# AY-Liu/Image-Editing-Framework

Measured on AMD Instinct MI355X. Metric: denoising steps/sec (SD1.5 512x512 P2P edit step, UNet batch 4), higher is better.
Workload: dtype f16x3; 1 GPU; sd15 UNet (859.5M params) P2P AttentionRefine edit step, 2 prompts x CFG = batch 4, 64x64 latents (512x512 px), 50-step DDIM, guidance 7.5, cross 0.8 / self 0.4, per-step null-text unconditional embeddings (P2P_NTI, edit_real.py); one independent edit per GPU; precision mode f16x3: fp32 storage; every contraction on split operands: hi + lo fp16 halves of each fp32 element, Ah Bh + Al Bh + Ah Bl =

## Files before the change

### image-editing-framework_amd/csrc/conv_halo_x3p.hip

```cpp
#include "x3p_common.h"

template <int N>
struct IntTag { static constexpr int value = N; };

template <bool UPS>
__global__ __launch_bounds__(768) void conv3x3_halo_x3p_kernel(const IefGemmX3pParams p) {
    constexpr int BM = 256, BN = 80, BK = XP_BK, NW = 8, NL = 4;
    constexpr int TM = 2, TN = 5;
    constexpr int WMAX = 64;
    constexpr int NPA = (BM + 2 * WMAX + 2 + 15) / 16;
    constexpr int APL = NPA * 1024;
    constexpr int AD = 2 * APL + 128;
    constexpr int ZA = 2 * APL;
    constexpr int NPB = BN / 16;
    constexpr int BPL = NPB * 1024, BBUF = 2 * BPL, NSB = 5;
    constexpr int BOFF = 2 * AD, DUMP = BOFF + NSB * BBUF;
    constexpr int LDS_BYTES = DUMP + 1024;
    constexpr int NU = 2 * NPA;
    constexpr int ATAPS = 5, APT = 3;
    static_assert(ATAPS * APT * NL >= NU && 3 * NL >= 2 * NPB, "loader schedule");
    static_assert(LDS_BYTES <= 160 * 1024, "LDS");
    __shared__ __attribute__((aligned(1024))) char smem[LDS_BYTES];

    const int tid = threadIdx.x, lane = tid & 63;
// ... 187 lines not shown
            one_step(IntTag<6>{}, IntTag<1>{}, abuf, abuf_n); one_step(IntTag<7>{}, IntTag<0>{}, abuf, abuf_n);
            one_step(IntTag<8>{}, IntTag<1>{}, abuf, abuf_n);
        }
    }
    asm volatile("s_waitcnt lgkmcnt(0)" ::: "memory");

    const float inv = p.inv_scale;
    if (p.splits > 1) {
        float* slab = p.ws + (long long)blockIdx.y * p.M * p.N;
#pragma unroll
        for (int i = 0; i < TM; ++i) {
            const int m = m0 + wave * 32 + i * 16 + fr;
            if (m >= p.M) continue;
#pragma unroll
            for (int j = 0; j < TN; ++j) {
                const int n = n0 + j * 16 + 4 * fq;
                if (n < p.N) *(f32x4*)(slab + (long long)m * p.N + n) = acc[j][i] * inv;
            }
        }
        return;
    }
#pragma unroll
    for (int i = 0; i < TM; ++i) {
        const int m = m0 + wave * 32 + i * 16 + fr;
        if (m >= p.M) continue;
#pragma unroll
        for (int j = 0; j < TN; ++j) {
            const int n = n0 + j * 16 + 4 * fq;
            if (n < p.N) xp_store(p, acc[j][i] * inv, m, n);
        }
    }
}

int ief_conv_halo_x3p_dispatch(const IefGemmX3pParams& p, hipStream_t st) {
    if (!p.conv || p.stride != 1 || p.pad_hi_only || p.CE1 || p.CE2 || p.Wd < 2 || p.H < 2 || p.geglu) return IEF_ESHAPE;
    if (p.ups) {
        if (p.tile != 12 || p.Wd > 128 || (p.H * p.Wd) % 256 || 256 % p.Wd) return IEF_ESHAPE;
    } else if (p.tile != 11 || p.Wd > 64) return IEF_ESHAPE;
    const int ncb = (p.C1 + p.C2) / XP_BK;
    if (p.splits > ncb) return IEF_ESHAPE;
    const int tiles = ((p.M + 255) / 256) * ((p.N + 79) / 80);
    const int splits = p.splits > 1 ? p.splits : 1;
    if (p.ups) hipLaunchKernelGGL(conv3x3_halo_x3p_kernel<true>, dim3(tiles, splits), dim3(768), 0, st, p);
    else hipLaunchKernelGGL(conv3x3_halo_x3p_kernel<false>, dim3(tiles, splits), dim3(768), 0, st, p);
    IEF_LAUNCH_CHECK();
    return IEF_OK;
}
```

### image-editing-framework_amd/csrc/gemm_x3p.hip

```cpp
#include "ief_common.h"
#include "ief_params.h"
#include "x3_common.h"

#include "x3p_common.h"

template <int BM, int BN, int WAVES_M, int WAVES_N, int NS, int NL, bool CONV>
__global__ __launch_bounds__(64 * (WAVES_M * WAVES_N + NL)) void igemm_x3p_kernel(const IefGemmX3pParams p) {
    constexpr int BK = XP_BK;
    constexpr int NWC = WAVES_M * WAVES_N;
    constexpr int NSW = NL > 0 ? NL : NWC;
    constexpr int PA = BM / 16, PB = BN / 16;
    constexpr int P = 2 * (PA + PB);
    constexpr int G = (P + NSW - 1) / NSW;
    constexpr int WM = BM / WAVES_M, WN = BN / WAVES_N, TM = WM / 16, TN = WN / 16;
    constexpr int SLOT = P * 16 * BK;
    constexpr int DUMP = NS * SLOT;
    static_assert(BM % 16 == 0 && BN % 16 == 0 && WM % 16 == 0 && WN % 16 == 0, "tile");
    static_assert(NS >= 2 && NS <= 4, "ring depth");
    static_assert((NS * SLOT + 512) * 2 <= 160 * 1024, "LDS");
    __shared__ __attribute__((aligned(1024))) half_t smem[NS * SLOT + 512];

    const int tid = threadIdx.x, lane = tid & 63;
    const int wave = __builtin_amdgcn_readfirstlane(tid >> 6);
    const int wr = wave / WAVES_N, wc = wave % WAVES_N;
// ... 388 lines not shown
        xp_store(p, a, m, n);
    }
}

__global__ __launch_bounds__(256) void x3_split_act_kernel(const float* __restrict__ x, half_t* __restrict__ planes, long long plane,
                                                           long long rows, int C4, int ldx, int ldp, float scale) {
    const long long total = rows * C4;
    for (long long i = (long long)blockIdx.x * 256 + threadIdx.x; i < total; i += (long long)gridDim.x * 256) {
        const long long r = i / C4;
        const int c = (int)(i - r * C4) * 4;
        half4 h, l;
        split4(*(const f32x4*)(x + r * ldx + c), scale, h, l);
        half_t* o = planes + r * ldp + c;
        *(half4*)o = h;
        *(half4*)(o + plane) = l;
    }
}
extern "C" int ief_x3_split_act(const float* x, ief_half* planes, long long plane, long long rows, int C, int ldx, int ldp, float scale,
                                void* stream) {
    if (!x || !planes) return IEF_EINVAL;
    if (rows <= 0 || C <= 0 || (C & 3) || (ldx & 3) || (ldp & 3) || (plane & 3) || !(scale > 0.f)) return IEF_ESHAPE;
    if (((uintptr_t)x & 15) || ((uintptr_t)planes & 7)) return IEF_EALIGN;
    long long grid = (rows * (C / 4) + 255) / 256;
    if (grid > 16384) grid = 16384;
    hipLaunchKernelGGL(x3_split_act_kernel, dim3((unsigned)grid), dim3(256), 0, (hipStream_t)stream, x, (half_t*)planes, plane, rows,
                       C / 4, ldx, ldp, scale);
    IEF_LAUNCH_CHECK();
    return IEF_OK;
}

extern "C" int ief_gemm_x3p_tile_bm(int tile) {
    switch (tile) {
        case 1: case 2: case 3: case 7: return 128;
        case 4: case 8: case 11: case 12: return 256;
        case 5: return 64;
        case 6: return 128;
        default: return 0;
    }
}
extern "C" int ief_gemm_x3p_tile_wn(int tile) { return tile == 6 ? 64 : tile == 8 ? 160 : 80; }
extern "C" int ief_gemm_x3p_tile_bn(int tile) {
    switch (tile) {
        case 1: case 2: case 4: case 5: case 7: return 160;
        case 3: case 11: case 12: return 80;
        case 6: return 64;
        case 8: return 320;
        default: return 0;
    }
}

template <int BM, int BN, int WAVES_M, int WAVES_N, int NS, int NL>
static int launch_x3p(const IefGemmX3pParams& p, hipStream_t st) {
    const int tiles = ((p.M + BM - 1) / BM) * ((p.N + BN - 1) / BN);
    const int splits = p.splits > 1 ? p.splits : 1;
    constexpr int NT = 64 * (WAVES_M * WAVES_N + NL);
    if (p.conv) hipLaunchKernelGGL((igemm_x3p_kernel<BM, BN, WAVES_M, WAVES_N, NS, NL, true>), dim3(tiles, splits), dim3(NT), 0, st, p);
    else hipLaunchKernelGGL((igemm_x3p_kernel<BM, BN, WAVES_M, WAVES_N, NS, NL, false>), dim3(tiles, splits), dim3(NT), 0, st, p);
    IEF_LAUNCH_CHECK();
    return IEF_OK;
}

int ief_conv_halo_x3p_dispatch(const IefGemmX3pParams& p, hipStream_t st);

extern "C" int ief_gemm_x3p(const IefGemmX3pParams* pp, void* stream) {
    if (!pp || !pp->A || !pp->W || !pp->zeros || (!pp->Out && !pp->OutP)) return IEF_EINVAL;
    IefGemmX3pParams p = *pp;
    if (p.M <= 0 || p.N <= 0 || p.K <= 0 || (p.K % XP_BK) || (p.N & 3)) return IEF_ESHAPE;
    if (p.rowvec && p.rows_per_batch <= 0) return IEF_ESHAPE;
    if (p.splits > 1 && (!p.ws || p.splits > 64 || p.geglu || p.rstat_out || p.cstat_out)) return IEF_EINVAL;
    if (!(p.inv_scale > 0.f)) return IEF_EINVAL;
    if ((p.ldw & 7) || (p.planeW & 7) || ((uintptr_t)p.W & 15)) return IEF_EALIGN;
    if (p.Out && ((p.ldo & 3) || ((uintptr_t)p.Out & 15))) return IEF_EALIGN;
    if (p.OutP && ((p.ldp & 3) || (p.planeO & 3) || ((uintptr_t)p.OutP & 7))) return IEF_EALIGN;
    if ((p.bias && ((uintptr_t)p.bias & 15)) || (p.rowvec && ((uintptr_t)p.rowvec & 15)) ||
        (p.residual && (((uintptr_t)p.residual & 15) || (p.ldr & 3)))) return IEF_EALIGN;
    if (p.geglu && ((p.N & 15) || p.residual || p.rowvec)) return IEF_EINVAL;
    if (p.rstat_out && (p.splits > 1 || p.geglu || p.tile == 11 || p.tile == 12 || (p.N % ief_gemm_x3p_tile_wn(p.tile)))) return IEF_EINVAL;
    if (p.rstat_in && (!p.colsum || p.rstat_slots <= 0 || p.rstat_cnt <= 0 || p.rstat_slots * p.rstat_cnt != p.K || p.splits > 1 ||
                       p.conv || !(p.ln_eps > 0.f) || ((uintptr_t)p.colsum & 15))) return IEF_EINVAL;
    if (p.conv) {
        if (p.C1 <= 0 || p.C2 < 0 || (p.C1 % XP_BK) || (p.C2 % XP_BK) || (p.CE1 % XP_BK) || (p.CE2 % XP_BK)) return IEF_ESHAPE;
        if ((p.C2 > 0 && !p.A2) || (p.CE1 > 0 && !p.E1) || (p.CE2 > 0 && !p.E2) || (p.CE2 > 0 && p.CE1 == 0)) return IEF_EINVAL;
        if (p.stride != 1 && p.stride != 2) return IEF_ESHAPE;
        if (p.ups != 0 && p.ups != 1) return IEF_ESHAPE;
        if (p.ups && ((p.H | p.Wd) & 1)) return IEF_ESHAPE;
        if ((p.CE1 + p.CE2) > 0 && (p.stride != 1 || p.ups)) return IEF_ESHAPE;
        if (p.K != 9 * (p.C1 + p.C2) + p.CE1 + p.CE2 || p.batch_images <= 0 || p.M != p.batch_images * p.Ho * p.Wo) return IEF_ESHAPE;
        const long long in_pix = (long long)p.batch_images * (p.H >> p.ups) * (p.Wd >> p.ups);
        const int cmax = p.C1 > p.C2 ? p.C1 : p.C2, emax = p.CE1 > p.CE2 ? p.CE1 : p.CE2;
        if (in_pix * cmax * 2 >= (1ll << 32) || (long long)p.M * emax * 2 >= (1ll << 32)) return IEF_ESHAPE;
        if (((uintptr_t)p.A & 15) || (p.planeA & 7) || (p.A2 && (((uintptr_t)p.A2 & 15) || (p.planeA2 & 7))) ||
            (p.E1 && (((uintptr_t)p.E1 & 15) || (p.planeE1 & 7))) || (p.E2 && (((uintptr_t)p.E2 & 15) || (p.planeE2 & 7)))) return IEF_EALIGN;
    } else {
        if ((p.lda & 7) || (p.planeA & 7) || ((uintptr_t)p.A & 15)) return IEF_EALIGN;
    }
    hipStream_t st = (hipStream_t)stream;
    int rc;
    switch (p.tile) {
        case 2: rc = launch_x3p<128, 160, 4, 2, 4, 4>(p, st); break;
        case 3: rc = launch_x3p<128, 80, 4, 1, 3, 0>(p, st); break;
        case 4: rc = launch_x3p<256, 160, 4, 2, 3, 0>(p, st); break;
        case 5: rc = launch_x3p<64, 160, 2, 2, 4, 0>(p, st); break;
        case 6: rc = launch_x3p<128, 64, 4, 1, 3, 0>(p, st); break;
        case 7: rc = launch_x3p<128, 160, 2, 2, 2, 0>(p, st); break;
        case 8: rc = launch_x3p<256, 320, 4, 2, 2, 0>(p, st); break;
        case 11: case 12: rc = ief_conv_halo_x3p_dispatch(p, st); break;
        case 1: default: rc = launch_x3p<128, 160, 4, 2, 4, 0>(p, st); break;
    }
    if (rc) return rc;
    if (p.splits > 1) {
        const long long total = (long long)p.M * (p.N / 4);
        int grid = (int)((total + 255) / 256);
        if (grid > 8192) grid = 8192;
        hipLaunchKernelGGL(x3p_reduce_kernel, dim3(grid), dim3(256), 0, st, p);
        IEF_LAUNCH_CHECK();
    }
    return IEF_OK;
}
```

### image-editing-framework_amd/csrc/split_x3.hip

```cpp
#include "ief_common.h"
#include "ief_params.h"

#include "x3_common.h"

__global__ __launch_bounds__(256) void x3_split_weights_kernel(const float* __restrict__ w, half_t* __restrict__ planes, long long n4,
                                                               float s) {
    for (long long i = (long long)blockIdx.x * 256 + threadIdx.x; i < n4; i += (long long)gridDim.x * 256) {
        half4 h, l;
        split4(((const f32x4*)w)[i], s, h, l);
        ((half4*)planes)[i] = h;
        ((half4*)planes)[n4 + i] = l;
    }
}
extern "C" int ief_x3_split_weights(const float* w, void* planes, long long n, float scale, void* stream) {
    if (!w || !planes) return IEF_EINVAL;
    if (n <= 0 || (n & 3) || !(scale > 0.f)) return IEF_ESHAPE;
    if (((uintptr_t)w & 15) || ((uintptr_t)planes & 7)) return IEF_EALIGN;
    long long grid = (n / 4 + 255) / 256;
    if (grid > 16384) grid = 16384;
    hipLaunchKernelGGL(x3_split_weights_kernel, dim3((unsigned)grid), dim3(256), 0, (hipStream_t)stream, w, (half_t*)planes, n / 4, scale);
    IEF_LAUNCH_CHECK();
    return IEF_OK;
}

template <int WM, int WN, int TM, int TN, int KIND, bool TRANSB, bool BPRE>
__global__ __launch_bounds__(64 * WM * WN, (2 * 2 * 16 * (WM * TM + WN * TN) * YLD * 2 > 80 * 1024) ? (WM * WN) / 4 : (WM * WN) / 2)
void igemm_x3_kernel(const IefGemmF32Params p) {
    constexpr bool CONV = KIND >= X3_CONV;
    constexpr bool HASFAST = KIND == X3_LIN || KIND == X3_CONV;
    constexpr int NTH = 64 * WM * WN;
    constexpr int BM = 16 * WM * TM, BN = 16 * WN * TN;
    constexpr int ROWS = BM + BN;
    constexpr int NA = (BM * 8 + NTH - 1) / NTH;
    constexpr int NBC = BPRE ? 2 * BN * 4 : BN * 8;
    constexpr int NB = (NBC + NTH - 1) / NTH;
    constexpr bool A_EXACT = (BM * 8) % NTH == 0, B_EXACT = NBC % NTH == 0;
    static_assert(!(BPRE && TRANSB), "pre-split planes are [N][K]");
    constexpr unsigned OOB = 0xFFFFFFF0u;
    constexpr unsigned OOBF = 0x80000000u;
    __shared__ __attribute__((aligned(16))) half_t smem_y[2 * 2 * ROWS * YLD];
    const int tid = threadIdx.x, lane = tid & 63, wid = tid >> 6;
    const int wm = wid / WN, wn = wid - wm * WN;
    const int lr = lane & 15, lg = lane >> 4;
    const int ntn = (p.N + BN - 1) / BN;
    const int ntiles = ((p.M + BM - 1) / BM) * ntn;
    const int bid = xcd_remap(blockIdx.x, ntiles);
    const int ntm = (p.M + BM - 1) / BM;
    const int grp = bid / (X3_GROUP_M * ntn), within = bid - grp * (X3_GROUP_M * ntn);
    const int gsz = min(X3_GROUP_M, ntm - grp * X3_GROUP_M);
    const int tn = within / gsz, tm = grp * X3_GROUP_M + (within - tn * gsz);
    const int m0 = tm * BM, n0 = tn * BN;
    const float* A = p.A;
    const float* W = p.W;
// ... 1088 lines not shown
```

### image-editing-framework_amd/hip.py

```python
import ctypes
import os
from ctypes import byref

import torch

from . import cabi

ABI_VERSION = cabi.defines["IEF_ABI_VERSION"]
REPEAT_MAX_JOBS = cabi.defines["IEF_REPEAT_MAX_JOBS"]
_LIB_PATH = os.environ.get("IEF_HIP_LIB") or os.path.join(os.path.dirname(os.path.abspath(__file__)), "libief_hip.so")
_lib = None


class HipExtensionMissing(RuntimeError):
    pass


IefGemmParams = cabi.structs["IefGemmParams"]
IefAttnParams = cabi.structs["IefAttnParams"]
IefCrossParams = cabi.structs["IefCrossParams"]
IefGemmF32Params = cabi.structs["IefGemmF32Params"]
IefAttnF32Params = cabi.structs["IefAttnF32Params"]
IefRepeatJob = cabi.structs["IefRepeatJob"]
IefGemmX3pParams = cabi.structs["IefGemmX3pParams"]
# ... 372 lines not shown
    def __init__(self, mode: str):
        if mode not in ("f32", "x3"):
            raise ValueError('f32_contraction: mode must be "f32" or "x3"')
        self.mode = mode

    def __enter__(self):
        global _F32_CONTRACT
        self.saved, _F32_CONTRACT = _F32_CONTRACT, self.mode
        return self

    def __exit__(self, *exc):
        global _F32_CONTRACT
        _F32_CONTRACT = self.saved
        return False


_x3_planes = {}
X3_FUSE_GEGLU = os.environ.get("IEF_X3_FUSE_GEGLU", "1") == "1"
X3_PRESPLIT = os.environ.get("IEF_X3_PRESPLIT", "1") == "1"


def x3_weight_planes(w, scale=None):
    scale = X3_SCALE_W if scale is None else scale
    key = (w.data_ptr(), tuple(w.shape), float(scale))
    hit = _x3_planes.get(key)
    if hit is not None and hit[0]() is w and hit[1] == w._version:
        return hit[2]
    if _capturing() or w.numel() % 4 or not w.is_contiguous():
        return None
    lib = load()
    n = w.shape[0]
    planes = torch.empty(2, n, w.numel() // n, dtype=torch.float16, device=w.device)
    _check(lib.ief_x3_split_weights(w.data_ptr(), planes.data_ptr(), w.numel(), float(scale), _stream()), "ief_x3_split_weights")
    import weakref
    _x3_planes[key] = (weakref.ref(w), w._version, planes)
    weakref.finalize(w, _x3_planes.pop, key, None)
    return planes


def _set_x3(p, sa, sb, w=None) -> str:
    if _F32_CONTRACT == "x3":
        p.x3, p.sa, p.sb = 1, sa, sb
        if w is not None and X3_PRESPLIT and (w.numel() // w.shape[0]) % 8 == 0:
            planes = x3_weight_planes(w, sb)
            if planes is not None:
                p._planes = planes
                p.Wp = planes.data_ptr()
        return "igemm_x3_kernel"
    return "igemm_f32_kernel"


def _is32(t) -> bool:
    return isinstance(t, torch.Tensor) and t.dtype == torch.float32


def _act32(t, name):
    if not (isinstance(t, torch.Tensor) and t.is_cuda and t.dtype == torch.float32):
        raise TypeError(f"{name}: expected an fp32 device tensor (reference-precision mode), got "
                        f"{type(t).__name__ if not isinstance(t, torch.Tensor) else (t.dtype, t.device)}")
    if t.stride(-1) != 1:
        raise ValueError(f"{name}: last dimension must be contiguous")
    return t


def _rows_ld32(t, name):
    _act32(t, name)
# ... 1555 lines not shown
```

### image-editing-framework_amd/planes.py

```python
import os
from ctypes import byref

import torch

from . import hip
from .hip import IefGemmX3pParams, _check, _dev32, _ptr, _stream, _Timed, _zeros

ACT_SCALE = 1.0
W_SCALE = hip.X3_SCALE_W


class Planes:
    __slots__ = ("t",)

    def __init__(self, t):
        if not (isinstance(t, torch.Tensor) and t.dtype == torch.float16 and t.dim() >= 2 and t.shape[0] == 2 and t.stride(-1) == 1):
            raise TypeError("Planes: expected an fp16 tensor [2, ...] with a contiguous last dimension")
        if not t.is_cuda:
            raise TypeError("Planes: device tensor expected (no CPU path)")
        self.t = t

    @staticmethod
    def empty(*shape, device):
        return Planes(torch.empty(2, *shape, dtype=torch.float16, device=device))
# ... 59 lines not shown
    return out


def weight_planes(w):
    t = hip.x3_weight_planes(w, W_SCALE)
    if t is None:
        raise RuntimeError("weight planes missing while capturing: run one eager forward first")
    return t


_PLAN_FILE = os.environ.get("IEF_PLAN_FILE_X3") or os.path.join(os.path.dirname(os.path.abspath(__file__)), "tuned_plans_x3.json")
_plans = None
TILE_FORCE = int(os.environ.get("IEF_X3P_TILE", "0"))


def _plan_table():
    global _plans
    if _plans is None:
        _plans = {}
        if os.path.exists(_PLAN_FILE) and os.environ.get("IEF_NO_PLAN_TABLE", "0") != "1":
            import json
            with open(_PLAN_FILE) as f:
                _plans = {k: tuple(v) for k, v in json.load(f).items()}
    return _plans


def save_plans(path=None):
    import json
    with open(path or _PLAN_FILE, "w") as f:
        json.dump({k: list(v) for k, v in sorted(_plan_table().items())}, f, indent=0)


_TILES = {1: (128, 160), 2: (128, 160), 3: (128, 80), 4: (256, 160), 5: (64, 160), 6: (128, 64), 7: (128, 160), 8: (256, 320),
          11: (256, 80), 12: (256, 80)}


def heuristic_plan(M, N, K, conv=False):
    nk = K // 32
    if N % 80 and N % 64 == 0:
        tile = 6
    elif N % 160:
        tile = 3
    elif M <= 64:
        tile = 5
    else:
        t1 = -(-M // 128) * (N // 160)
        tile = 4 if t1 >= 1024 and M % 256 == 0 else 1
    bm, bn = _TILES[tile]
    tiles = -(-M // bm) * -(-N // bn)
    splits = 1
    if tiles < 160 and nk >= 16:
        splits = max(1, min(-(-256 // tiles), nk // 8, 16))
    return tile, splits


def pick_plan(M, N, K, conv=False, variant=""):
    hit = _plan_table().get(f"{'conv' if conv else 'gemm'}|{M}|{N}|{K}{variant}")
    if hit is None:
        hit = heuristic_plan(M, N, K, conv)
    if TILE_FORCE and (TILE_FORCE < 10 or conv):
        return TILE_FORCE, hit[1]
    return hit[0], hit[1]


AUTOTUNE = os.environ.get("IEF_AUTOTUNE_X3", "0") == "1"


def candidate_plans(M, N, K, conv=False, halo_ok=False, ncb=0, geglu=False):
    nk = K // 32
    out = []
    for t, (bm, bn) in _TILES.items():
        if t in (11, 12):
            continue
        if N % bn or (t == 6 and N % 80 == 0):
            continue
        tiles = -(-M // bm) * (N // bn)
        for sp in (1, 2, 3, 4, 6, 8, 12, 16):
            if sp > 1 and (geglu or nk // sp < 4 or tiles * sp > 2048 or tiles >= 512):
                continue
            if tiles * sp < 40 and sp < 16:
                continue
            out.append((t, sp))
    if conv and halo_ok:
        tiles = -(-M // 256) * (N // 80)
        for sp in (1, 2, 3, 4, 5, 6, 8, 10, 12, 16, 20):
            if sp > 1 and (sp > ncb // 2 or tiles * sp > 1024 or tiles >= 384):
                continue
            if tiles * sp < 40 and sp < 16:
                continue
            out.append((11, sp))
    return out


def _autotune(key, cands, run, w):
    wc = hip._cold_copies(w)
    for x in wc:
        weight_planes(x)
    best = None
    for t, sp in cands:
        try:
            us = hip._time_graph(lambda i: run(t, sp, wc[i % len(wc)]))
        except (RuntimeError, ValueError):
            continue
        if best is None or us < best[0]:
            best = (us, t, sp)
    for x in wc[1:]:
        hip._x3_planes.pop((x.data_ptr(), tuple(x.shape), float(W_SCALE)), None)
    if best is not None:
        _plan_table()[key] = (best[1], best[2])
    return best


def supported(N, K):
    return (N % 80 == 0 or N % 64 == 0) and K % 32 == 0


def _out_args(p, M, No, out, out_planes, device, lead_shape):
    o32 = op = None
    if out is True or isinstance(out, torch.Tensor) or (out is None and out_planes in (None, False)):
        o32 = out if isinstance(out, torch.Tensor) else torch.empty(*lead_shape, No, dtype=torch.float32, device=device)
        Mo, Nn, ldo = hip._rows_ld32(o32, "out")
        if (Mo, Nn) != (M, No):
            raise ValueError("x3p: out shape mismatch")
        p.Out, p.ldo = o32.data_ptr(), ldo
    if out_planes not in (None, False):
        op = out_planes if isinstance(out_planes, Planes) else Planes.empty(*lead_shape, No, device=device)
        Mp, Np, ldp = op.rows_ld("out_planes")
        if (Mp, Np) != (M, No):
            raise ValueError("x3p: out_planes shape mismatch")
        p.OutP, p.planeO, p.ldp = op.t.data_ptr(), op.plane, ldp
    return o32, op


def _ret(o32, op):
    if o32 is not None and op is not None:
        return o32, op
    return o32 if op is None else op


class RowStats:
# ... 80 lines not shown
        _check(lib.ief_gemm_x3p(byref(p), _stream()), "ief_gemm_x3p")
    r = _ret(o32, op)
    if row_stats:
        return (r + (rs,)) if isinstance(r, tuple) else (r, rs)
    return r


def conv3x3(x, w, bias=None, x2=None, stride=1, upsample=False, rowvec=None, residual=None, out=None, out_planes=None,
            extra=None, pad_hi_only=False, tile=0, splits=0):
    lib = hip.load()
    if not isinstance(x, Planes) or (x2 is not None and not isinstance(x2, Planes)):
        raise TypeError("planes.conv3x3: x / x2 must be Planes")
    if not x.is_contiguous() or (x2 is not None and not x2.is_contiguous()) or not w.is_contiguous():
        raise ValueError("planes.conv3x3: x, x2, w must be contiguous")
    B, Hp, Wp, C1 = x.shape
    C2 = 0 if x2 is None else x2.shape[-1]
    Cout = w.shape[0]
    e1 = e2 = None
    CE1 = CE2 = 0
    if extra is not None:
        e1, e2 = extra
        CE1 = e1.shape[-1]
        CE2 = 0 if e2 is None else e2.shape[-1]
        for e in (e1, e2):
            if e is not None and (not isinstance(e, Planes) or not e.is_contiguous() or tuple(e.shape[:3]) != (B, Hp, Wp)):
                raise ValueError("planes.conv3x3: extra sources must be contiguous NHWC Planes at the output resolution")
    K = 9 * (C1 + C2) + CE1 + CE2
    if w.numel() != Cout * K:
        raise ValueError(f"planes.conv3x3: weight {tuple(w.shape)} does not match K = {K}")
    H, Wd = (Hp * 2, Wp * 2) if upsample else (Hp, Wp)
    pad_total = 1 if pad_hi_only else 2
    Ho, Wo = (H + pad_total - 3) // stride + 1, (Wd + pad_total - 3) // stride + 1
    M = B * Ho * Wo
    wp = weight_planes(w)
    p = IefGemmX3pParams()
    p.A, p.planeA = x.t.data_ptr(), x.plane
    if x2 is not None:
        p.A2, p.planeA2 = x2.t.data_ptr(), x2.plane
    if e1 is not None:
        p.E1, p.planeE1 = e1.t.data_ptr(), e1.plane
    if e2 is not None:
        p.E2, p.planeE2 = e2.t.data_ptr(), e2.plane
    p.W, p.planeW, p.ldw = wp.data_ptr(), wp.stride(0), K
    o32, op = _out_args(p, M, Cout, out, out_planes, x.device, (B, Ho, Wo))
    p.bias = _ptr(_dev32(bias, "bias")) if bias is not None else None
    if rowvec is not None:
        _dev32(rowvec, "rowvec")
        if rowvec.dim() != 2 or rowvec.shape[1] != Cout or rowvec.shape[0] not in (1, B):
            raise ValueError("planes.conv3x3: rowvec must be [B, Cout] or [1, Cout]")
        p.rowvec = rowvec.data_ptr()
        p.rows_per_batch = Ho * Wo if rowvec.shape[0] == B and B > 1 else B * Ho * Wo
    if residual is not None:
        if tuple(hip._act32(residual, "residual").shape) != (B, Ho, Wo, Cout) or not residual.is_contiguous():
            raise ValueError("planes.conv3x3: residual must be contiguous fp32 [B, Ho, Wo, Cout]")
        p.residual, p.ldr = residual.data_ptr(), Cout
    p.M, p.N, p.K = M, Cout, K
    p.conv, p.H, p.Wd, p.C1, p.C2, p.Ho, p.Wo = 1, H, Wd, C1, C2, Ho, Wo
    p.stride, p.ups, p.batch_images, p.pad_hi_only = stride, 1 if upsample else 0, B, 1 if pad_hi_only else 0
    p.CE1, p.CE2 = CE1, CE2
    p.out_scale, p.inv_scale, p.zeros = 1.0, 1.0 / (ACT_SCALE * W_SCALE), _zeros(x.device)
    halo_ok = HALO and stride == 1 and not pad_hi_only and extra is None and Hp >= 2 and Cout % 80 == 0 and (
        (not upsample and 2 <= Wd <= 64) or (upsample and Wd <= 128 and (H * Wd) % 256 == 0 and 256 % Wd == 0))
    if tile:
        p.tile, p.splits = tile, max(1, splits)
    else:
        variant = ("|u" if upsample else "") + (f"|s{stride}" if stride != 1 else "") + ("|e" if extra is not None else "")
        key = f"conv|{M}|{Cout}|{K}{variant}"
        if AUTOTUNE and key not in _plan_table() and not hip._capturing() and hip._prof is None:
            _autotune(key, candidate_plans(M, Cout, K, conv=True, halo_ok=halo_ok, ncb=(C1 + C2) // 32),
                      lambda t, sp, wi: conv3x3(x, wi, bias, x2=x2, stride=stride, upsample=upsample, rowvec=rowvec, residual=residual,
                                                out=out, out_planes=out_planes, extra=extra, pad_hi_only=pad_hi_only, tile=t, splits=sp), w)
        hit = _plan_table().get(key)
        if hit is not None and (hit[0] not in (11, 12) or halo_ok):
            p.tile, p.splits = hit[0], hit[1]
        elif halo_ok:
            tiles, ncb = -(-M // 256) * (Cout // 80), (C1 + C2) // 32
            sp = 1
            while tiles * sp < 192 and sp * 2 <= ncb // 2 and sp < 16:
                sp *= 2
            p.tile, p.splits = 11, sp
        else:
            p.tile, p.splits = heuristic_plan(M, Cout, K, conv=True)
            if TILE_FORCE and TILE_FORCE < 10:
                p.tile = TILE_FORCE
    if p.tile in (11, 12):
        if not halo_ok:
            raise ValueError("planes.conv3x3: this geometry has no halo form (tile 11 / 12)")
        p.tile = 12 if upsample else 11
        p.splits = min(p.splits, (C1 + C2) // 32)
    ws = None
    if p.splits > 1:
        ws = torch.empty(p.splits * M * Cout, dtype=torch.float32, device=x.device)
        p.ws = ws.data_ptr()
    nbytes = 4.0 * (B * Hp * Wp * (C1 + C2) + M * (CE1 + CE2) + Cout * K + M * Cout * ((1 if o32 is not None else 0) + (1 if op is not None else 0) + (1 if residual is not None else 0)))
    kn = f"conv3x3_halo_x3p_kernel<{'true' if upsample else 'false'}>" if p.tile in (11, 12) else f"igemm_x3p_kernel<true> t{p.tile}"
    kn += f" {M}x{Cout}x{K} s{p.splits}" if hip.PROF_SHAPES else ""
    if p.tile in (11, 12):
        hip.note_staged(kn, 4.0 * (C1 + C2) * (9 * 80 + 256 + 2 * (Wd + 1)) * -(-M // 256) * -(-Cout // 80))
    else:
        bm, bn = _TILES[p.tile]
        hip.note_staged(kn, 4.0 * K * (bm + bn) * -(-M // bm) * -(-Cout // bn))
    with _Timed(kn, 2.0 * M * Cout * K, nbytes):
        _check(lib.ief_gemm_x3p(byref(p), _stream()), "ief_gemm_x3p (conv)")
    return _ret(o32, op)


GN_SMALL_ELEMS = int(os.environ.get("IEF_GN_SMALL_ELEMS", str(3 << 20)))
GN_REG_MAX_HW = int(os.environ.get("IEF_GN_REG_MAX_HW", "1024"))
HALO = os.environ.get("IEF_X3P_HALO", "1") == "1"
ENABLED = os.environ.get("IEF_X3P", "1") == "1"


def groupnorm(x, gamma, beta, groups, eps, silu=False, x2=None, out32=False):
    lib = hip.load()
    if not hip._act32(x, "x").is_contiguous() or (x2 is not None and not hip._act32(x2, "x2").is_contiguous()):
        raise ValueError("planes.groupnorm: inputs must be contiguous")
    B, C1 = x.shape[0], x.shape[-1]
    C2 = 0 if x2 is None else x2.shape[-1]
    HW = x.numel() // (B * C1)
    out = Planes.empty(*x.shape[:-1], C1 + C2, device=x.device)
    cpg = (C1 + C2) // groups
    if HW <= GN_REG_MAX_HW and lib.ief_groupnorm_reg_fits(C1, C2, HW, groups):
        o32 = torch.empty(*x.shape[:-1], C1 + C2, dtype=torch.float32, device=x.device) if out32 else None
        with _Timed("groupnorm_reg_kernel", 0.0, (12.0 if out32 else 8.0) * (x.numel() + (0 if x2 is None else x2.numel()))):
            _check(lib.ief_groupnorm_silu_reg(x.data_ptr(), _ptr(x2), C1, C2, _ptr(o32), out.t.data_ptr(), out.plane,
                                              _dev32(gamma, "gamma").data_ptr(), _dev32(beta, "beta").data_ptr(), B, HW, groups,
                                              eps, 1 if silu else 0, _stream()), "ief_groupnorm_silu_reg")
        return (out, o32) if out32 else out
    if not out32 and HW <= GN_REG_MAX_HW and B * HW * (C1 + C2) <= GN_SMALL_ELEMS and cpg % 2 == 0 and C1 % 2 == 0 and cpg // 2 <= 256:
        with _Timed("groupnorm_f32_kernel", 0.0, 12.0 * (x.numel() + (0 if x2 is None else x2.numel()))):
# ... 194 lines not shown
```

### include/ief_hip.h

```cpp
#ifndef IEF_HIP_H
#define IEF_HIP_H
#include <stdint.h>

#ifdef __HIPCC__
typedef _Float16 ief_half;
#else
typedef uint16_t ief_half;
#endif

#ifdef __cplusplus
extern "C" {
#endif

#define IEF_ABI_VERSION 4
int ief_abi_version(void);
const char* ief_target_arch(void);
int ief_struct_size(int which);

typedef struct IefGemmParams {
    const ief_half* A;
    const ief_half* A2;
    const ief_half* W;
    ief_half* Out;
    const float* bias;
// ... 188 lines not shown
int ief_repeat_batch(const IefRepeatJob* jobs, int njobs, void* stream);
int ief_image_u8(const float* x, unsigned char* out, int B, int C, int H, int Wd, void* stream);

typedef struct IefGemmX3pParams {
    const ief_half* A;  long long planeA;
    const ief_half* A2; long long planeA2;
    const ief_half* E1; long long planeE1;
    const ief_half* E2; long long planeE2;
    const ief_half* W;  long long planeW;
    float* Out;
    ief_half* OutP; long long planeO;
    const float* bias;
    const float* rowvec;
    const float* residual;
    int M, N, K;
    int lda, ldw, ldo, ldp, ldr;
    int conv, H, Wd, C1, C2, Ho, Wo, stride, ups, batch_images, pad_hi_only, CE1, CE2;
    int rows_per_batch;
    float out_scale;
    float inv_scale;
    int tile;
    int splits;
    float* ws;
    int geglu;
    const void* zeros;
    float* rstat_out;
    float* cstat_out;
    const float* rstat_in;
    const float* colsum;
    int rstat_slots, rstat_cnt;
    float ln_eps;
} IefGemmX3pParams;
int ief_gemm_x3p(const IefGemmX3pParams* p, void* stream);
int ief_gemm_x3p_tile_bm(int tile);
int ief_gemm_x3p_tile_bn(int tile);
int ief_gemm_x3p_tile_wn(int tile);
int ief_x3_split_act(const float* x, ief_half* planes, long long plane, long long rows, int C, int ldx, int ldp, float scale,
                     void* stream);

int ief_groupnorm_bwd_f32(const float* x, const float* x2, int C1, int C2, const float* dy, const float* add, float* dx, float* dx2,
                          const float* gamma, const float* beta, int B, int HW, int groups, float eps, int silu, void* stream);
int ief_layernorm_bwd_f32(const float* x, const float* dy, const float* add, float* dx, const float* gamma, long long rows, int C,
                          float eps, void* stream);
int ief_geglu_il_bwd_f32(const float* pre, const float* dy, float* dpre, long long rows, int Ch, void* stream);
int ief_zero_insert2x_f32(const float* in, float* out, int B, int H, int W, int C, void* stream);
int ief_pool2x2_sum_f32(const float* in, float* out, int B, int H, int W, int C, void* stream);
int ief_conv_out_bwd_f32w(const float* d_eps, const float* w, float* dh, int B, int C, int H, int W, int Cout, void* stream);
int ief_softmax_bwd_rows_f32(const float* P, float* dP, long long rows, int L, float scale, void* stream);
int ief_transpose_batched_f32(const float* in, float* out, int R, int N, int L, void* stream);
int ief_map_loss_rows_blocks(long long rows);
int ief_map_loss_rows_f32(const float* P, const float* ref, float* dP, float* loss, long long rows, int L, float gcoef,
                          float loss_coef, void* stream);
int ief_nti_adam_f32g(float* param, float* m, float* v, const float* grad, const float* stats, const float* hyper, int* step, int n,
                      void* stream);

typedef struct IefAttnBwdParams {
    const ief_half* Q; const ief_half* K; const ief_half* V; const ief_half* dO;
    const float* lse;
    const float* delta;
    ief_half* dQ; ief_half* dK; ief_half* dV;
    int B, heads, N, L, d;
    int ldq, ldk, ldv, ldo, lddq, lddk, lddv;
    float scale;
    float ds_mul;
    int kv_splits;
    float* ws;
// ... 60 lines not shown
```

Baseline: 74.67 steps/s.

## Add polyphase 2x2 conv kernel for nearest-upsample 3x3 convolutions

Adds a tile-13 path that rewrites nearest-2x-upsample followed by a 3x3 conv as four output phases. Each phase is a 2x2 conv on the low-resolution input, using weights pre-summed per phase. This cuts the contraction from 9 taps to 4 per channel block and avoids reading the upsampled halo. A new kernel precomputes and caches the phase weight planes. The path is reachable only through autotune or a plan-table entry, and the summed weights change fp32 rounding slightly.

```diff
diff --git a/image-editing-framework_amd/csrc/conv_halo_x3p.hip b/image-editing-framework_amd/csrc/conv_halo_x3p.hip
--- a/image-editing-framework_amd/csrc/conv_halo_x3p.hip
+++ b/image-editing-framework_amd/csrc/conv_halo_x3p.hip
@@ -243,8 +243,228 @@
     }
 }
 
+__global__ __launch_bounds__(768) void conv3x3_halo_x3p_kernel_phase(const IefGemmX3pParams p) {
+    constexpr int BM = 256, BN = 80, BK = XP_BK, NW = 8, NL = 4;
+    constexpr int TM = 2, TN = 5;
+    constexpr int WMAX = 64;
+    constexpr int NPA = (BM + 2 * WMAX + 2 + 15) / 16;
+    constexpr int APL = NPA * 1024;
+    constexpr int AD = 2 * APL + 128;
+    constexpr int ZA = 2 * APL;
+    constexpr int NPB = BN / 16;
+    constexpr int BPL = NPB * 1024, BBUF = 2 * BPL, NSB = 5;
+    constexpr int BOFF = 2 * AD, DUMP = BOFF + NSB * BBUF;
+    constexpr int LDS_BYTES = DUMP + 1024;
+    constexpr int NU = 2 * NPA;
+    constexpr int NT = 4;
+    constexpr int APT = (NU + NL - 1) / NL;
+    static_assert(APT * NL >= NU && 3 * NL >= 2 * NPB, "loader schedule");
+    static_assert(LDS_BYTES <= 160 * 1024, "LDS");
+    __shared__ __attribute__((aligned(1024))) char smem[LDS_BYTES];
+
+    const int tid = threadIdx.x, lane = tid & 63;
+    const int wave = __builtin_amdgcn_readfirstlane(tid >> 6);
+    const int W = p.Wd >> 1, H = p.H >> 1;
+    const int Ms = p.batch_images * H * W;
+    const int tiles_n = (p.N + BN - 1) / BN, tiles_m = (Ms + BM - 1) / BM;
+    const int lid = xcd_remap(blockIdx.x, gridDim.x);
+    const int grp = lid / (XP_GROUP_M * tiles_n), within = lid - grp * (XP_GROUP_M * tiles_n);
+    const int gsz = min(XP_GROUP_M, tiles_m - grp * XP_GROUP_M);
+    const int tn = within / gsz, tm = grp * XP_GROUP_M + (within - tn * gsz);
+    const int m0 = tm * BM, n0 = tn * BN;
+    const int py = (int)blockIdx.z >> 1, px = (int)blockIdx.z & 1;
+    const int Ctot = p.C1 + p.C2;
+    const char* __restrict__ zp = (const char*)p.zeros;
+    const int st_row0 = m0 - (W + 1);
+
+    const int ncb = Ctot / BK;
+    int cb_lo = 0, cb_hi = ncb;
+    if (p.splits > 1) {
+        const int per = (ncb + p.splits - 1) / p.splits;
+        cb_lo = min(ncb, (int)blockIdx.y * per);
+        cb_hi = min(ncb, cb_lo + per);
+    }
+    const int nblk = cb_hi - cb_lo;
+
+    if (tid < 16) { ((float*)(smem + ZA))[tid] = 0.f; ((float*)(smem + ZA + AD))[tid] = 0.f; }
+    asm volatile("s_waitcnt lgkmcnt(0)" ::: "memory");
+
+    if (wave >= NW) {
+        const int l = wave - NW;
+        const unsigned st_chunk = (unsigned)(XP_LANE_CHUNK(lane) * 16);
+        const int ms_lane = st_row0 + (lane >> 2);
+        const char* an_src = zp; long long an_pl = 0; unsigned an_cs = 0, an_c0 = 0; bool an_on = false;
+        auto set_next_block = [&](int cb, bool on) {
+            const bool first = cb * BK < p.C1;
+            an_src = (const char*)(first ? p.A : p.A2);
+            an_pl = (first ? p.planeA : p.planeA2) * 2;
+            an_cs = (unsigned)(first ? p.C1 : p.C2);
+            an_c0 = (unsigned)(first ? cb * BK : cb * BK - p.C1);
+            an_on = on;
+        };
+        auto issue_a = [&](int u, int buf_off) {
+            const bool exists = u < NU;
+            const int pl = u >= NPA ? 1 : 0, q = u - pl * NPA;
+            const int ms = ms_lane + 16 * q;
+            const bool ok = exists && an_on && (unsigned)ms < (unsigned)Ms;
+            const char* g = ok ? an_src + ((long long)pl * an_pl + (long long)((unsigned)ms * an_cs + an_c0) * 2 + st_chunk) : zp;
+            glds16(g, (half_t*)(smem + (exists ? pl * AD + buf_off + q * 1024 : DUMP)));
+        };
+        const long long w_lane = ((long long)blockIdx.z * p.N + n0 + (lane >> 2)) * p.K * 2 + st_chunk;
+        auto issue_b = [&](int cb, int tap, bool on, int slot_off) {
+            const long long k0 = (long long)(tap * Ctot + cb * BK) * 2;
+#pragma unroll
+            for (int j = 0; j < 3; ++j) {
+                const int v = l + NL * j;
+                const bool exists = v < 2 * NPB;
+                const int pl = v >= NPB ? 1 : 0, q = v - pl * NPB;
+                const bool ok = exists && on && n0 + 16 * q + (lane >> 2) < p.N;
+                const char* g = ok ? (const char*)p.W + ((long long)pl * p.planeW * 2 + w_lane + (long long)(16 * q) * p.K * 2 + k0) : zp;
+                glds16(g, (half_t*)(smem + (exists ? BOFF + slot_off + pl * BPL + q * 1024 : DUMP)));
+            }
+        };
+        auto n_issued = [](int tap) constexpr -> int { return 3 + (tap == 0 ? APT : 0); };
+        if (nblk > 0) {
+            set_next_block(cb_lo, true);
+#pragma unroll
+            for (int j = 0; j < APT; ++j) issue_a(l + NL * j, 0);
+            issue_b(cb_lo, 0, true, 0);
+            issue_b(cb_lo, 1, true, BBUF);
+            issue_b(cb_lo, 2, true, 2 * BBUF);
+            issue_b(cb_lo, 3, true, 3 * BBUF);
+            asm volatile("s_waitcnt vmcnt(9)" ::: "memory");
+            XP_BARRIER();
+        }
+        int bs_prev = 4 * BBUF, bs = 0, bs_next = BBUF;
+        for (int cbi = 0; cbi < nblk; ++cbi) {
+            const int cb = cb_lo + cbi;
+            const int abuf_n = APL - (cbi & 1) * APL;
+            const bool more = cb + 1 < cb_hi;
+            set_next_block(min(cb + 1, cb_hi - 1), more);
+            auto one_step = [&](auto tap_tag) {
+                constexpr int tap = decltype(tap_tag)::value;
+                asm volatile("s_waitcnt vmcnt(%0)" ::"n"(n_issued((tap + NT - 1) % NT) + n_issued((tap + NT - 2) % NT)) : "memory");
+                XP_BARRIER();
+                if constexpr (tap == 0) {
+#pragma unroll
+                    for (int j = 0; j < APT; ++j) issue_a(l + NL * j, abuf_n);
+                }
+                issue_b(cb + 1, tap, more, bs_prev);
+                bs_prev = bs; bs = bs_next; bs_next = bs_next == (NSB - 1) * BBUF ? 0 : bs_next + BBUF;
+            };
+            one_step(IntTag<0>{}); one_step(IntTag<1>{}); one_step(IntTag<2>{}); one_step(IntTag<3>{});
+        }
+        asm volatile("s_waitcnt vmcnt(0)" ::: "memory");
+        return;
+    }
+
+    const int fr = lane & 15, fq = lane >> 4;
+    int a_off[TM][NT];
+    int m_out[TM];
+#pragma unroll
+    for (int i = 0; i < TM; ++i) {
+        const int r = wave * 32 + i * 16 + fr, m = m0 + r;
+        const int img = m / (H * W), rem = m - img * (H * W);
+        const int y = rem / W, x = rem - y * W;
+        m_out[i] = m < Ms ? (img * 2 * H + 2 * y + py) * (2 * W) + 2 * x + px : -1;
+#pragma unroll
+        for (int s = 0; s < NT; ++s) {
+            const int ty = py + (s >> 1), tx = px + (s & 1);
+            const bool zero = m >= Ms || (tx == 0 && x == 0) || (tx == 2 && x == W - 1) || (ty == 0 && y == 0) || (ty == 2 && y == H - 1);
+            const int sr = r + ty * W + tx;
+            a_off[i][s] = zero ? -1 : sr * 64 + ((fq ^ xp_swz(sr)) << 4);
+        }
+    }
+    int b_off[TN];
+#pragma unroll
+    for (int j = 0; j < TN; ++j) {
+        const int row = j * 16 + fr;
+        b_off[j] = BOFF + row * 64 + ((fq ^ xp_swz(row)) << 4);
+    }
+    f32x4 acc[TN][TM];
+#pragma unroll
+    for (int j = 0; j < TN; ++j)
+#pragma unroll
+        for (int i = 0; i < TM; ++i) acc[j][i] = f32x4{0.f, 0.f, 0.f, 0.f};
+
+    half8 ah[2][TM], al[2][TM], bh[TN], bl[TN];
+    auto read_a = [&](half8 (&h)[TM], half8 (&l)[TM], int abuf, auto tap_tag) {
+        constexpr int s = decltype(tap_tag)::value;
+#pragma unroll
+        for (int i = 0; i < TM; ++i) {
+            const int ad = a_off[i][s] < 0 ? ZA : abuf + a_off[i][s];
+            h[i] = *(const half8*)(smem + ad);
+            l[i] = *(const half8*)(smem + ad + AD);
+        }
+    };
+    if (nblk > 0) {
+        XP_BARRIER();
+        read_a(ah[0], al[0], 0, IntTag<0>{});
+#pragma unroll
+        for (int j = 0; j < TN; ++j) { bh[j] = *(const half8*)(smem + b_off[j]); bl[j] = *(const half8*)(smem + b_off[j] + BPL); }
+    }
+    int bs_next = BBUF;
+    auto one_step = [&](auto tap_tag, int abuf, int abuf_n) {
+        constexpr int tap = decltype(tap_tag)::value, PAR = tap & 1;
+        XP_BARRIER();
+        read_a(ah[PAR ^ 1], al[PAR ^ 1], tap == NT - 1 ? abuf_n : abuf, IntTag<(tap + 1) % NT>{});
+#pragma unroll
+        for (int j = 0; j < TN; ++j) {
+#pragma unroll
+            for (int i = 0; i < TM; ++i) {
+                acc[j][i] = __builtin_amdgcn_mfma_f32_16x16x32_f16(bl[j], ah[PAR][i], acc[j][i], 0, 0, 0);
+                acc[j][i] = __builtin_amdgcn_mfma_f32_16x16x32_f16(bh[j], al[PAR][i], acc[j][i], 0, 0, 0);
+                acc[j][i] = __builtin_amdgcn_mfma_f32_16x16x32_f16(bh[j], ah[PAR][i], acc[j][i], 0, 0, 0);
+            }
+            bh[j] = *(const half8*)(smem + bs_next + b_off[j]);
+            bl[j] = *(const half8*)(smem + bs_next + b_off[j] + BPL);
+        }
+        bs_next = bs_next == (NSB - 1) * BBUF ? 0 : bs_next + BBUF;
+    };
+    for (int cbi = 0; cbi < nblk; ++cbi) {
+        const int abuf = (cbi & 1) * APL, abuf_n = APL - abuf;
+        one_step(IntTag<0>{}, abuf, abuf_n); one_step(IntTag<1>{}, abuf, abuf_n);
+        one_step(IntTag<2>{}, abuf, abuf_n); one_step(IntTag<3>{}, abuf, abuf_n);
+    }
+    asm volatile("s_waitcnt lgkmcnt(0)" ::: "memory");
+
+    const float inv = p.inv_scale;
+    if (p.splits > 1) {
+        float* slab = p.ws + (long long)blockIdx.y * p.M * p.N;
+#pragma unroll
+        for (int i = 0; i < TM; ++i) {
+            if (m_out[i] < 0) continue;
+#pragma unroll
+            for (int j = 0; j < TN; ++j) {
+                const int n = n0 + j * 16 + 4 * fq;
+                if (n < p.N) *(f32x4*)(slab + (long long)m_out[i] * p.N + n) = acc[j][i] * inv;
+            }
+        }
+        return;
+    }
+#pragma unroll
+    for (int i = 0; i < TM; ++i) {
+        if (m_out[i] < 0) continue;
+#pragma unroll
+        for (int j = 0; j < TN; ++j) {
+            const int n = n0 + j * 16 + 4 * fq;
+            if (n < p.N) xp_store(p, acc[j][i] * inv, m_out[i], n);
+        }
+    }
+}
+
 int ief_conv_halo_x3p_dispatch(const IefGemmX3pParams& p, hipStream_t st) {
     if (!p.conv || p.stride != 1 || p.pad_hi_only || p.CE1 || p.CE2 || p.Wd < 2 || p.H < 2 || p.geglu) return IEF_ESHAPE;
+    if (p.tile == 13) {
+        const int Wi = p.Wd >> 1, Hi = p.H >> 1;
+        if (!p.ups || Wi > 64 || Wi < 2 || Hi < 2 || p.K != 4 * (p.C1 + p.C2) || p.ldw != p.K) return IEF_ESHAPE;
+        const int ncb = (p.C1 + p.C2) / XP_BK;
+        if (p.splits > ncb) return IEF_ESHAPE;
+        const int tiles = ((p.M / 4 + 255) / 256) * ((p.N + 79) / 80);
+        hipLaunchKernelGGL(conv3x3_halo_x3p_kernel_phase, dim3(tiles, p.splits > 1 ? p.splits : 1, 4), dim3(768), 0, st, p);
+        IEF_LAUNCH_CHECK();
+        return IEF_OK;
+    }
     if (p.ups) {
         if (p.tile != 12 || p.Wd > 128 || (p.H * p.Wd) % 256 || 256 % p.Wd) return IEF_ESHAPE;
     } else if (p.tile != 11 || p.Wd > 64) return IEF_ESHAPE;
diff --git a/image-editing-framework_amd/csrc/gemm_x3p.hip b/image-editing-framework_amd/csrc/gemm_x3p.hip
--- a/image-editing-framework_amd/csrc/gemm_x3p.hip
+++ b/image-editing-framework_amd/csrc/gemm_x3p.hip
@@ -444,7 +444,7 @@
 extern "C" int ief_gemm_x3p_tile_bm(int tile) {
     switch (tile) {
         case 1: case 2: case 3: case 7: return 128;
-        case 4: case 8: case 11: case 12: return 256;
+        case 4: case 8: case 11: case 12: case 13: return 256;
         case 5: return 64;
         case 6: return 128;
         default: return 0;
@@ -454,7 +454,7 @@
 extern "C" int ief_gemm_x3p_tile_bn(int tile) {
     switch (tile) {
         case 1: case 2: case 4: case 5: case 7: return 160;
-        case 3: case 11: case 12: return 80;
+        case 3: case 11: case 12: case 13: return 80;
         case 6: return 64;
         case 8: return 320;
         default: return 0;
@@ -487,7 +487,7 @@
     if ((p.bias && ((uintptr_t)p.bias & 15)) || (p.rowvec && ((uintptr_t)p.rowvec & 15)) ||
         (p.residual && (((uintptr_t)p.residual & 15) || (p.ldr & 3)))) return IEF_EALIGN;
     if (p.geglu && ((p.N & 15) || p.residual || p.rowvec)) return IEF_EINVAL;
-    if (p.rstat_out && (p.splits > 1 || p.geglu || p.tile == 11 || p.tile == 12 || (p.N % ief_gemm_x3p_tile_wn(p.tile)))) return IEF_EINVAL;
+    if (p.rstat_out && (p.splits > 1 || p.geglu || p.tile == 11 || p.tile == 12 || p.tile == 13 || (p.N % ief_gemm_x3p_tile_wn(p.tile)))) return IEF_EINVAL;
     if (p.rstat_in && (!p.colsum || p.rstat_slots <= 0 || p.rstat_cnt <= 0 || p.rstat_slots * p.rstat_cnt != p.K || p.splits > 1 ||
                        p.conv || !(p.ln_eps > 0.f) || ((uintptr_t)p.colsum & 15))) return IEF_EINVAL;
     if (p.conv) {
@@ -497,7 +497,8 @@
         if (p.ups != 0 && p.ups != 1) return IEF_ESHAPE;
         if (p.ups && ((p.H | p.Wd) & 1)) return IEF_ESHAPE;
         if ((p.CE1 + p.CE2) > 0 && (p.stride != 1 || p.ups)) return IEF_ESHAPE;
-        if (p.K != 9 * (p.C1 + p.C2) + p.CE1 + p.CE2 || p.batch_images <= 0 || p.M != p.batch_images * p.Ho * p.Wo) return IEF_ESHAPE;
+        const int ktaps = p.tile == 13 ? 4 : 9;
+        if (p.K != ktaps * (p.C1 + p.C2) + p.CE1 + p.CE2 || p.batch_images <= 0 || p.M != p.batch_images * p.Ho * p.Wo) return IEF_ESHAPE;
         const long long in_pix = (long long)p.batch_images * (p.H >> p.ups) * (p.Wd >> p.ups);
         const int cmax = p.C1 > p.C2 ? p.C1 : p.C2, emax = p.CE1 > p.CE2 ? p.CE1 : p.CE2;
         if (in_pix * cmax * 2 >= (1ll << 32) || (long long)p.M * emax * 2 >= (1ll << 32)) return IEF_ESHAPE;
@@ -516,7 +517,7 @@
         case 6: rc = launch_x3p<128, 64, 4, 1, 3, 0>(p, st); break;
         case 7: rc = launch_x3p<128, 160, 2, 2, 2, 0>(p, st); break;
         case 8: rc = launch_x3p<256, 320, 4, 2, 2, 0>(p, st); break;
-        case 11: case 12: rc = ief_conv_halo_x3p_dispatch(p, st); break;
+        case 11: case 12: case 13: rc = ief_conv_halo_x3p_dispatch(p, st); break;
         case 1: default: rc = launch_x3p<128, 160, 4, 2, 4, 0>(p, st); break;
     }
     if (rc) return rc;
diff --git a/image-editing-framework_amd/csrc/split_x3.hip b/image-editing-framework_amd/csrc/split_x3.hip
--- a/image-editing-framework_amd/csrc/split_x3.hip
+++ b/image-editing-framework_amd/csrc/split_x3.hip
@@ -19,6 +19,41 @@
     long long grid = (n / 4 + 255) / 256;
     if (grid > 16384) grid = 16384;
     hipLaunchKernelGGL(x3_split_weights_kernel, dim3((unsigned)grid), dim3(256), 0, (hipStream_t)stream, w, (half_t*)planes, n / 4, scale);
+    IEF_LAUNCH_CHECK();
+    return IEF_OK;
+}
+
+__global__ __launch_bounds__(256) void x3_upsample_phase_weights_kernel(const float* __restrict__ w, half_t* __restrict__ planes, int Cout,
+                                                                        int C4, float s) {
+    const long long n4 = 16ll * Cout * C4;
+    for (long long i = (long long)blockIdx.x * 256 + threadIdx.x; i < n4; i += (long long)gridDim.x * 256) {
+        const int c4 = (int)(i % C4);
+        long long r = i / C4;
+        const int tap = (int)(r & 3);
+        r >>= 2;
+        const int n = (int)(r % Cout), ph = (int)(r / Cout);
+        const int py = ph >> 1, px = ph & 1, sy = tap >> 1, sx = tap & 1;
+        const int ky0 = py ? 2 * sy : sy, ky1 = py ? 1 + sy : 2 * sy;
+        const int kx0 = px ? 2 * sx : sx, kx1 = px ? 1 + sx : 2 * sx;
+        const f32x4* src = (const f32x4*)w + (long long)n * 9 * C4 + c4;
+        f32x4 a = src[(ky0 * 3 + kx0) * C4];
+        for (int ky = ky0; ky <= ky1; ++ky)
+            for (int kx = kx0; kx <= kx1; ++kx)
+                if (ky != ky0 || kx != kx0) a = a + src[(ky * 3 + kx) * C4];
+        half4 h, l;
+        split4(a, s, h, l);
+        ((half4*)planes)[i] = h;
+        ((half4*)planes)[n4 + i] = l;
+    }
+}
+extern "C" int ief_x3_upsample_phase_weights(const float* w, void* planes, int Cout, int C, float scale, void* stream) {
+    if (!w || !planes) return IEF_EINVAL;
+    if (Cout <= 0 || C <= 0 || (C & 3) || !(scale > 0.f)) return IEF_ESHAPE;
+    if (((uintptr_t)w & 15) || ((uintptr_t)planes & 7)) return IEF_EALIGN;
+    long long grid = (16ll * Cout * (C / 4) + 255) / 256;
+    if (grid > 16384) grid = 16384;
+    hipLaunchKernelGGL(x3_upsample_phase_weights_kernel, dim3((unsigned)grid), dim3(256), 0, (hipStream_t)stream, w, (half_t*)planes, Cout,
+                       C / 4, scale);
     IEF_LAUNCH_CHECK();
     return IEF_OK;
 }
diff --git a/image-editing-framework_amd/hip.py b/image-editing-framework_amd/hip.py
--- a/image-editing-framework_amd/hip.py
+++ b/image-editing-framework_amd/hip.py
@@ -428,6 +428,26 @@
     n = w.shape[0]
     planes = torch.empty(2, n, w.numel() // n, dtype=torch.float16, device=w.device)
     _check(lib.ief_x3_split_weights(w.data_ptr(), planes.data_ptr(), w.numel(), float(scale), _stream()), "ief_x3_split_weights")
+    import weakref
+    _x3_planes[key] = (weakref.ref(w), w._version, planes)
+    weakref.finalize(w, _x3_planes.pop, key, None)
+    return planes
+
+
+def x3_upsample_phase_planes(w, scale=None):
+    scale = X3_SCALE_W if scale is None else scale
+    key = (w.data_ptr(), tuple(w.shape), float(scale), "phase")
+    hit = _x3_planes.get(key)
+    if hit is not None and hit[0]() is w and hit[1] == w._version:
+        return hit[2]
+    if _capturing() or not w.is_contiguous():
+        return None
+    if w.dim() != 4 or tuple(w.shape[1:3]) != (3, 3) or w.shape[3] % 4:
+        raise ValueError("x3_upsample_phase_planes: weight must be [Cout, 3, 3, C] with C a multiple of 4")
+    lib = load()
+    n, c = w.shape[0], w.shape[3]
+    planes = torch.empty(2, 4, n, 4 * c, dtype=torch.float16, device=w.device)
+    _check(lib.ief_x3_upsample_phase_weights(w.data_ptr(), planes.data_ptr(), n, c, float(scale), _stream()), "ief_x3_upsample_phase_weights")
     import weakref
     _x3_planes[key] = (weakref.ref(w), w._version, planes)
     weakref.finalize(w, _x3_planes.pop, key, None)
diff --git a/image-editing-framework_amd/planes.py b/image-editing-framework_amd/planes.py
--- a/image-editing-framework_amd/planes.py
+++ b/image-editing-framework_amd/planes.py
@@ -115,7 +115,8 @@
 
 
 _TILES = {1: (128, 160), 2: (128, 160), 3: (128, 80), 4: (256, 160), 5: (64, 160), 6: (128, 64), 7: (128, 160), 8: (256, 320),
-          11: (256, 80), 12: (256, 80)}
+          11: (256, 80), 12: (256, 80), 13: (256, 80)}
+_HALO = (11, 12, 13)
 
 
 def heuristic_plan(M, N, K, conv=False):
@@ -149,11 +150,11 @@
 AUTOTUNE = os.environ.get("IEF_AUTOTUNE_X3", "0") == "1"
 
 
-def candidate_plans(M, N, K, conv=False, halo_ok=False, ncb=0, geglu=False):
+def candidate_plans(M, N, K, conv=False, halo_ok=False, ncb=0, geglu=False, phase_ok=False):
     nk = K // 32
     out = []
     for t, (bm, bn) in _TILES.items():
-        if t in (11, 12):
+        if t in _HALO:
             continue
         if N % bn or (t == 6 and N % 80 == 0):
             continue
@@ -172,6 +173,14 @@
             if tiles * sp < 40 and sp < 16:
                 continue
             out.append((11, sp))
+    if conv and phase_ok:
+        tiles = -(-(M // 4) // 256) * (N // 80) * 4
+        for sp in (1, 2, 3, 4, 5, 6, 8, 10, 12, 16, 20):
+            if sp > 1 and (sp > ncb // 2 or tiles * sp > 1024 or tiles >= 384):
+                continue
+            if tiles * sp < 40 and sp < 16:
+                continue
+            out.append((13, sp))
     return out
 
 
@@ -179,6 +188,8 @@
     wc = hip._cold_copies(w)
     for x in wc:
         weight_planes(x)
+        if any(t == 13 for t, _ in cands):
+            hip.x3_upsample_phase_planes(x, W_SCALE)
     best = None
     for t, sp in cands:
         try:
@@ -189,6 +200,7 @@
             best = (us, t, sp)
     for x in wc[1:]:
         hip._x3_planes.pop((x.data_ptr(), tuple(x.shape), float(W_SCALE)), None)
+        hip._x3_planes.pop((x.data_ptr(), tuple(x.shape), float(W_SCALE), "phase"), None)
     if best is not None:
         _plan_table()[key] = (best[1], best[2])
     return best
@@ -335,7 +347,6 @@
     pad_total = 1 if pad_hi_only else 2
     Ho, Wo = (H + pad_total - 3) // stride + 1, (Wd + pad_total - 3) // stride + 1
     M = B * Ho * Wo
-    wp = weight_planes(w)
     p = IefGemmX3pParams()
     p.A, p.planeA = x.t.data_ptr(), x.plane
     if x2 is not None:
@@ -344,7 +355,6 @@
         p.E1, p.planeE1 = e1.t.data_ptr(), e1.plane
     if e2 is not None:
         p.E2, p.planeE2 = e2.t.data_ptr(), e2.plane
-    p.W, p.planeW, p.ldw = wp.data_ptr(), wp.stride(0), K
     o32, op = _out_args(p, M, Cout, out, out_planes, x.device, (B, Ho, Wo))
     p.bias = _ptr(_dev32(bias, "bias")) if bias is not None else None
     if rowvec is not None:
@@ -364,17 +374,18 @@
     p.out_scale, p.inv_scale, p.zeros = 1.0, 1.0 / (ACT_SCALE * W_SCALE), _zeros(x.device)
     halo_ok = HALO and stride == 1 and not pad_hi_only and extra is None and Hp >= 2 and Cout % 80 == 0 and (
         (not upsample and 2 <= Wd <= 64) or (upsample and Wd <= 128 and (H * Wd) % 256 == 0 and 256 % Wd == 0))
+    phase_ok = HALO and upsample and stride == 1 and not pad_hi_only and extra is None and Hp >= 2 and 2 <= Wp <= 64 and Cout % 80 == 0
     if tile:
         p.tile, p.splits = tile, max(1, splits)
     else:
         variant = ("|u" if upsample else "") + (f"|s{stride}" if stride != 1 else "") + ("|e" if extra is not None else "")
         key = f"conv|{M}|{Cout}|{K}{variant}"
         if AUTOTUNE and key not in _plan_table() and not hip._capturing() and hip._prof is None:
-            _autotune(key, candidate_plans(M, Cout, K, conv=True, halo_ok=halo_ok, ncb=(C1 + C2) // 32),
+            _autotune(key, candidate_plans(M, Cout, K, conv=True, halo_ok=halo_ok, ncb=(C1 + C2) // 32, phase_ok=phase_ok),
                       lambda t, sp, wi: conv3x3(x, wi, bias, x2=x2, stride=stride, upsample=upsample, rowvec=rowvec, residual=residual,
                                                 out=out, out_planes=out_planes, extra=extra, pad_hi_only=pad_hi_only, tile=t, splits=sp), w)
         hit = _plan_table().get(key)
-        if hit is not None and (hit[0] not in (11, 12) or halo_ok):
+        if hit is not None and (hit[0] not in _HALO or (phase_ok if hit[0] == 13 else halo_ok)):
             p.tile, p.splits = hit[0], hit[1]
         elif halo_ok:
             tiles, ncb = -(-M // 256) * (Cout // 80), (C1 + C2) // 32
@@ -386,19 +397,34 @@
             p.tile, p.splits = heuristic_plan(M, Cout, K, conv=True)
             if TILE_FORCE and TILE_FORCE < 10:
                 p.tile = TILE_FORCE
-    if p.tile in (11, 12):
-        if not halo_ok:
-            raise ValueError("planes.conv3x3: this geometry has no halo form (tile 11 / 12)")
-        p.tile = 12 if upsample else 11
+    if p.tile == 13:
+        if not phase_ok:
+            raise ValueError("planes.conv3x3: this geometry has no phase form (tile 13)")
         p.splits = min(p.splits, (C1 + C2) // 32)
+        wp = hip.x3_upsample_phase_planes(w, W_SCALE)
+        if wp is None:
+            raise RuntimeError("phase weight planes missing while capturing: run one eager forward first")
+        K = 4 * (C1 + C2)
+        p.K = K
+    else:
+        if p.tile in (11, 12):
+            if not halo_ok:
+                raise ValueError("planes.conv3x3: this geometry has no halo form (tile 11 / 12)")
+            p.tile = 12 if upsample else 11
+            p.splits = min(p.splits, (C1 + C2) // 32)
+        wp = weight_planes(w)
+    p.W, p.planeW, p.ldw = wp.data_ptr(), wp.stride(0), K
     ws = None
     if p.splits > 1:
         ws = torch.empty(p.splits * M * Cout, dtype=torch.float32, device=x.device)
         p.ws = ws.data_ptr()
     nbytes = 4.0 * (B * Hp * Wp * (C1 + C2) + M * (CE1 + CE2) + Cout * K + M * Cout * ((1 if o32 is not None else 0) + (1 if op is not None else 0) + (1 if residual is not None else 0)))
-    kn = f"conv3x3_halo_x3p_kernel<{'true' if upsample else 'false'}>" if p.tile in (11, 12) else f"igemm_x3p_kernel<true> t{p.tile}"
+    kn = "conv3x3_halo_x3p_kernel_phase" if p.tile == 13 else \
+        f"conv3x3_halo_x3p_kernel<{'true' if upsample else 'false'}>" if p.tile in (11, 12) else f"igemm_x3p_kernel<true> t{p.tile}"
     kn += f" {M}x{Cout}x{K} s{p.splits}" if hip.PROF_SHAPES else ""
-    if p.tile in (11, 12):
+    if p.tile == 13:
+        hip.note_staged(kn, 4.0 * (C1 + C2) * (4 * 80 + 256 + 2 * (Wp + 1)) * -(-(M // 4) // 256) * -(-Cout // 80) * 4)
+    elif p.tile in (11, 12):
         hip.note_staged(kn, 4.0 * (C1 + C2) * (9 * 80 + 256 + 2 * (Wd + 1)) * -(-M // 256) * -(-Cout // 80))
     else:
         bm, bn = _TILES[p.tile]
diff --git a/include/ief_hip.h b/include/ief_hip.h
--- a/include/ief_hip.h
+++ b/include/ief_hip.h
@@ -244,6 +244,7 @@
     float ln_eps;
 } IefGemmX3pParams;
 int ief_gemm_x3p(const IefGemmX3pParams* p, void* stream);
+int ief_x3_upsample_phase_weights(const float* w, void* planes, int Cout, int C, float scale, void* stream);
 int ief_gemm_x3p_tile_bm(int tile);
 int ief_gemm_x3p_tile_bn(int tile);
 int ief_gemm_x3p_tile_wn(int tile);
```

New measurement: 76.34 steps/s (median of 6 runs). 1.02x the previous value.
